# AssemblyAI-Community/MinImagen

Hardware: NVIDIA H100
Metric: denoising steps/sec (SR256 U-Net, batch 32 per GPU per step) (higher is better)
Workload: dtype f16 tensor-core operands, f32 accumulate / residual stream

## Files before the change

### minimagen_b200/csrc/conv_tc.cu

```cuda
#include "conv_tc.cuh"

#include <cuda_runtime.h>
#include <mutex>
#include <stdio.h>

#include "kernels.cuh"
#include "launch.cuh"
#include "ptx.cuh"
#include "sat_half.cuh"
#include "wgmma.cuh"

namespace mi {

namespace {

constexpr int kNumThreads = 384;
constexpr uint32_t kABytes = kConvBlockM * kConvBlockK * 2;
constexpr uint32_t kRingBudget = 192 * 1024;
constexpr uint32_t kAuxBytes = 512;
constexpr uint32_t kSmemMax = 227 * 1024;
constexpr int kProducerRegs = 40;
constexpr int kConsumerRegs = 232;
static_assert(128 * kProducerRegs + 256 * kConsumerRegs <= 65536, "register file overcommitted");

template <int BLOCK_N>
struct Cfg {
    static constexpr uint32_t kBBytes = BLOCK_N * kConvBlockK * 2;
    static constexpr uint32_t kStageBytes = kABytes + kBBytes;
    static constexpr int kStages = (kRingBudget / kStageBytes) > 8 ? 8 : (kRingBudget / kStageBytes);
    static constexpr uint32_t kSmemBytes = kStages * kStageBytes + 1024  + kAuxBytes;
};

__device__ __forceinline__ float silu(float v) { return __fdividef(v, 1.0f + __expf(-v)); }

template <int BLOCK_N, bool GN>
__global__ void __launch_bounds__(kNumThreads, 1)
conv_wg_kernel(const __grid_constant__ CUtensorMap tmA, const __grid_constant__ CUtensorMap tmA2,
               const __grid_constant__ CUtensorMap tmB, const __grid_constant__ CUtensorMap tmX,
               const __grid_constant__ CUtensorMap tmX2, const __grid_constant__ ConvTcArgs args,
               const __grid_constant__ GnPrologueArgs gn) {
    using C = Cfg<BLOCK_N>;
    constexpr int STAGES = C::kStages;
    static_assert(2 * STAGES * 8 <= 256, "barrier block overlaps the GroupNorm scratch");

    extern __shared__ uint8_t smem_raw[];
    uint8_t* smem = reinterpret_cast<uint8_t*>((reinterpret_cast<uintptr_t>(smem_raw) + 1023) & ~uintptr_t(1023));
    uint64_t* bars = reinterpret_cast<uint64_t*>(smem + STAGES * C::kStageBytes);
    uint64_t* full_bar = bars;
    uint64_t* empty_bar = bars + STAGES;

    const int warp = threadIdx.x >> 5;
    const int lane = threadIdx.x & 31;
    const int wg = threadIdx.x >> 7;
    int* err = args.err_flag;

    if (threadIdx.x == 0) {
        ptx::prefetch_tensormap(&tmB);
        if (!GN) {
            ptx::prefetch_tensormap(&tmA);
            ptx::prefetch_tensormap(&tmA2);
        }
        for (int i = 0; i < STAGES; ++i) {
            ptx::mbar_init(&full_bar[i], GN ? 5 : 1);
            ptx::mbar_init(&empty_bar[i], 2);
        }
        ptx::fence_barrier_init();
    }
    __syncthreads();
    pdl_wait();

    const int num_tap_kb = args.num_taps * args.chunks_per_tap;
    const int num_kb = num_tap_kb + args.x_chunks;
    const int tiles_m = args.tiles_w * args.tiles_h * args.tiles_b;
    const int total_tiles = tiles_m * args.tiles_n;
    const int BW = 1 << args.bw_log2, BH = 1 << args.bh_log2;
    const int BB = kConvBlockM >> (args.bw_log2 + args.bh_log2);

    if (wg == 0) {
        if constexpr (!GN) {
            ptx::setmaxnreg_dec<kProducerRegs>();
            if (warp == 0) {
                int stage = 0;
                uint32_t phase = 0;
                for (int tile = blockIdx.x; tile < total_tiles; tile += gridDim.x) {
                    const int nt = tile % args.tiles_n;
                    const int mt = tile / args.tiles_n;
                    const int w0 = (mt % args.tiles_w) * BW;
                    const int h0 = ((mt / args.tiles_w) % args.tiles_h) * BH;
                    const int b0 = (mt / (args.tiles_w * args.tiles_h)) * BB;
                    const int n0 = nt * BLOCK_N;
                    for (int kb = 0; kb < num_kb; ++kb) {
                        ptx::mbar_wait(&empty_bar[stage], phase ^ 1, err, 100 + stage);
                        if (ptx::elect_one()) {
                            uint8_t* sa = smem + stage * C::kStageBytes;
                            uint8_t* sb = sa + kABytes;
                            ptx::mbar_arrive_expect_tx(&full_bar[stage], C::kStageBytes);
                            if (kb < num_tap_kb) {
                                const int t = kb / args.chunks_per_tap, j = kb - t * args.chunks_per_tap;
                                const int cw = w0 * args.in_stride + args.dw[t], ch = h0 * args.in_stride + args.dh[t];
                                if (j < args.a_split)
                                    ptx::tma_load_5d(&tmA, &full_bar[stage], sa, args.a_chan_off + j * kConvBlockK, cw, ch,
                                                     args.ph[t], b0);
                                else
                                    ptx::tma_load_5d(&tmA2, &full_bar[stage], sa,
                                                     args.a_chan_off2 + (j - args.a_split) * kConvBlockK, cw, ch, args.ph[t], b0);
                            } else {
                                const int jx = kb - num_tap_kb;
                                if (jx < args.x_split)
                                    ptx::tma_load_5d(&tmX, &full_bar[stage], sa, args.x_chan_off + jx * kConvBlockK, w0, h0, 0, b0);
                                else
                                    ptx::tma_load_5d(&tmX2, &full_bar[stage], sa,
                                                     args.x_chan_off2 + (jx - args.x_split) * kConvBlockK, w0, h0, 0, b0);
                            }
                            ptx::tma_load_2d(&tmB, &full_bar[stage], sb, kb * kConvBlockK, n0);
                        }
                        if (++stage == STAGES) { stage = 0; phase ^= 1; }
                    }
                }
                pdl_trigger();
            }
        } else {
            float* s_mean = reinterpret_cast<float*>(reinterpret_cast<uint8_t*>(bars) + 256);
            float* s_rstd = s_mean + 32;
            float* sA = reinterpret_cast<float*>(reinterpret_cast<uint8_t*>(bars) + kAuxBytes);
            const int tt = threadIdx.x;
            const int lq = tt & 7;
            const int prow = tt >> 3;
            const int C0 = gn.C0, C1 = gn.C1, Ctot = C0 + C1, Cg = Ctot / gn.groups;
            const int H = args.H, W = args.W;
            float* sB = sA + Ctot;
            int stage = 0;
            uint32_t phase = 0;
            int cur_b = -1;
            for (int tile = blockIdx.x; tile < total_tiles; tile += gridDim.x) {
                const int nt = tile % args.tiles_n;
                const int mt = tile / args.tiles_n;
                const int w0 = (mt % args.tiles_w) * BW;
                const int h0 = ((mt / args.tiles_w) % args.tiles_h) * BH;
                const int b = mt / (args.tiles_w * args.tiles_h);
                const int n0 = nt * BLOCK_N;
                if (b != cur_b) {
                    ptx::bar_sync(1, 128);
                    if (tt < gn.groups) {
                        const int g = tt;
                        double su = 0.0, sq = 0.0;
                        const int lo = g * Cg, hi = lo + Cg;
                        const int lo0 = min(lo, C0), hi0 = min(hi, C0);
                        for (int e = lo0 / 16; e < hi0 / 16; ++e) {
                            su += gn.stats0[((long long)b * (C0 / 16) + e) * 2];
                            sq += gn.stats0[((long long)b * (C0 / 16) + e) * 2 + 1];
                        }
                        const int lo1 = max(lo, C0) - C0, hi1 = max(hi, C0) - C0;
                        for (int e = lo1 / 16; e < hi1 / 16; ++e) {
                            su += (double)gn.scale1 * gn.stats1[((long long)b * (C1 / 16) + e) * 2];
                            sq += (double)gn.scale1 * (double)gn.scale1 * gn.stats1[((long long)b * (C1 / 16) + e) * 2 + 1];
                        }
                        const double n = (double)Cg * H * W;
                        const double mean = su / n;
                        double var = sq / n - mean * mean;
                        if (var < 0) var = 0;
                        s_mean[g] = (float)mean;
                        s_rstd[g] = (float)(1.0 / sqrt(var + (double)gn.eps));
                    }
                    ptx::bar_sync(1, 128);
                    for (int cc = tt; cc < Ctot; cc += 128) {
                        const int g = cc / Cg;
                        float a = s_rstd[g] * gn.gamma[cc];
                        float bb = gn.beta[cc] - s_mean[g] * a;
                        if (gn.scale_shift) {
                            const float sc = gn.scale_shift[(long long)b * gn.ss_ld + cc] + 1.0f;
                            const float shv = gn.scale_shift[(long long)b * gn.ss_ld + Ctot + cc];
                            a *= sc;
                            bb = bb * sc + shv;
                        }
                        if (cc >= C0) a *= gn.scale1;
                        sA[cc] = a;
                        sB[cc] = bb;
                    }
                    cur_b = b;
                    ptx::bar_sync(1, 128);
                }
                const long long img = (long long)b * H * W;
                for (int kb = 0; kb < num_kb; ++kb) {
                    const int t = kb / args.chunks_per_tap, j = kb - t * args.chunks_per_tap;
                    const int dh = args.dh[t], dw = args.dw[t];
                    const float* cA = sA + j * kConvBlockK + lq * 8;
                    const float* cB = sB + j * kConvBlockK + lq * 8;
                    const float4 a0 = *reinterpret_cast<const float4*>(cA), a1 = *reinterpret_cast<const float4*>(cA + 4);
                    const float4 b0 = *reinterpret_cast<const float4*>(cB), b1 = *reinterpret_cast<const float4*>(cB + 4);
                    const bool first = j < args.a_split;
                    const int Cs = first ? C0 : C1;
                    const float* src = (first ? gn.src0 + (long long)j * kConvBlockK
                                              : gn.src1 + (long long)(j - args.a_split) * kConvBlockK) + img * Cs + lq * 8;

                    ptx::mbar_wait(&empty_bar[stage], phase ^ 1, err, 600 + stage);
                    uint8_t* sa = smem + stage * C::kStageBytes;
                    if (warp == 0 && ptx::elect_one()) {
                        ptx::mbar_arrive_expect_tx(&full_bar[stage], C::kBBytes);
                        ptx::tma_load_2d(&tmB, &full_bar[stage], sa + kABytes, kb * kConvBlockK, n0);
                    }
                    float4 x0[8], x1[8];
                    bool ok[8];
#pragma unroll
                    for (int i = 0; i < 8; ++i) {
                        const int m = i * 16 + prow;
                        const int gw = w0 + (m & (BW - 1)) + dw;
                        const int gh = h0 + ((m >> args.bw_log2) & (BH - 1)) + dh;
                        ok[i] = gh >= 0 && gh < H && gw >= 0 && gw < W;
                        if (ok[i]) {
                            const float4* s4 = reinterpret_cast<const float4*>(src + ((long long)gh * W + gw) * Cs);
                            x0[i] = __ldg(s4);
                            x1[i] = __ldg(s4 + 1);
                        }
                    }
#pragma unroll
                    for (int i = 0; i < 8; ++i) {
                        const int m = i * 16 + prow;
                        uint4 o = make_uint4(0u, 0u, 0u, 0u);
                        if (ok[i]) {
                            const __half2 h0_ = sat_half2(silu(fmaf(x0[i].x, a0.x, b0.x)), silu(fmaf(x0[i].y, a0.y, b0.y)));
                            const __half2 h1_ = sat_half2(silu(fmaf(x0[i].z, a0.z, b0.z)), silu(fmaf(x0[i].w, a0.w, b0.w)));
                            const __half2 h2_ = sat_half2(silu(fmaf(x1[i].x, a1.x, b1.x)), silu(fmaf(x1[i].y, a1.y, b1.y)));
                            const __half2 h3_ = sat_half2(silu(fmaf(x1[i].z, a1.z, b1.z)), silu(fmaf(x1[i].w, a1.w, b1.w)));
                            o.x = *reinterpret_cast<const uint32_t*>(&h0_); o.y = *reinterpret_cast<const uint32_t*>(&h1_);
                            o.z = *reinterpret_cast<const uint32_t*>(&h2_); o.w = *reinterpret_cast<const uint32_t*>(&h3_);
                        }
                        *reinterpret_cast<uint4*>(sa + m * 128 + ((lq ^ (m & 7)) << 4)) = o;
                    }
                    ptx::fence_proxy_async_smem();
                    __syncwarp();
                    if (lane == 0) ptx::mbar_arrive(&full_bar[stage]);
                    if (++stage == STAGES) { stage = 0; phase ^= 1; }
                }
            }
            pdl_trigger();
        }
    } else {
        if constexpr (!GN) ptx::setmaxnreg_inc<kConsumerRegs>();
        const int cw = wg - 1;
        const int wq = warp & 3;
        const int cq = 2 * (lane & 3);
        float acc[BLOCK_N / 2];
        int stage = 0;
        uint32_t phase = 0;
        int m_r[2], bw_r[2], bh_r[2], bb_r[2];
#pragma unroll
        for (int r = 0; r < 2; ++r) {
            m_r[r] = cw * 64 + wq * 16 + (lane >> 2) + 8 * r;
            bw_r[r] = m_r[r] & (BW - 1);
            bh_r[r] = (m_r[r] >> args.bw_log2) & (BH - 1);
            bb_r[r] = m_r[r] >> (args.bw_log2 + args.bh_log2);
        }
        const int m_warp = cw * 64 + wq * 16;
        const int bb_warp = m_warp >> (args.bw_log2 + args.bh_log2);
        const bool vec = args.out_sc == 1 && ((reinterpret_cast<uintptr_t>(args.out_f32) & 7) == 0) &&
                         ((reinterpret_cast<uintptr_t>(args.residual) & 7) == 0) &&
                         ((reinterpret_cast<uintptr_t>(args.out_f16) & 3) == 0);

        for (int tile = blockIdx.x; tile < total_tiles; tile += gridDim.x) {
            const int nt = tile % args.tiles_n;
            const int mt = tile / args.tiles_n;
            const int n0 = nt * BLOCK_N;
            int prev = -1;
            for (int kb = 0; kb < num_kb; ++kb) {
                ptx::mbar_wait(&full_bar[stage], phase, err, 300 + stage);
                const uint32_t sa = ptx::smem_u32(smem + stage * C::kStageBytes);
                const uint64_t da = ptx::make_sw128_desc(sa + cw * (64 * 128));
                const uint64_t db = ptx::make_sw128_desc(sa + kABytes);
                ptx::wg_fence();
#pragma unroll
                for (int k = 0; k < kConvBlockK / 16; ++k)
                    ptx::Wgmma<BLOCK_N, 0>::run(acc, da + 2 * k, db + 2 * k, (kb | k) != 0);
                ptx::wg_commit();
                ptx::wg_wait<1>();
                if (prev >= 0 && (threadIdx.x & 127) == 0) ptx::mbar_arrive(&empty_bar[prev]);
                prev = stage;
                if (++stage == STAGES) { stage = 0; phase ^= 1; }
            }
            ptx::wg_wait<0>();
            ptx::wg_fence_regs(acc);
            if (prev >= 0 && (threadIdx.x & 127) == 0) ptx::mbar_arrive(&empty_bar[prev]);

            const int tw0 = (mt % args.tiles_w) * BW;
            const int th0 = ((mt / args.tiles_w) % args.tiles_h) * BH;
            const int tb0 = (mt / (args.tiles_w * args.tiles_h)) * BB;
            bool valid[2];
            long long pix[2];
#pragma unroll
            for (int r = 0; r < 2; ++r) {
                const int w = tw0 + bw_r[r], h = th0 + bh_r[r], b = tb0 + bb_r[r];
                valid[r] = (b < args.B) && (h < args.H) && (w < args.W);
                pix[r] = (long long)b * args.out_sb + (long long)h * args.out_sh + (long long)w * args.out_sw;
            }
            const bool fast = vec && n0 + BLOCK_N <= args.n_valid;
            float st_s[BLOCK_N / 16 > 0 ? BLOCK_N / 16 : 1], st_q[BLOCK_N / 16 > 0 ? BLOCK_N / 16 : 1];
#pragma unroll
            for (int q = 0; q < BLOCK_N / 16; ++q) { st_s[q] = 0.f; st_q[q] = 0.f; }
#pragma unroll
            for (int j = 0; j < BLOCK_N / 8; ++j) {
                const int n = n0 + 8 * j + cq;
                if (fast) {
                    float2 bv = make_float2(0.f, 0.f);
                    if (args.bias) bv = __ldg(reinterpret_cast<const float2*>(args.bias + n));
#pragma unroll
                    for (int r = 0; r < 2; ++r) {
                        if (!valid[r]) continue;
                        const long long o = pix[r] + n;
                        float2 f = make_float2(acc[4 * j + 2 * r] + bv.x, acc[4 * j + 2 * r + 1] + bv.y);
                        if (args.residual) {
                            const float2 rv = *reinterpret_cast<const float2*>(args.residual + o);
                            f.x += rv.x; f.y += rv.y;
                        }
                        st_s[j >> 1] += f.x + f.y;
                        st_q[j >> 1] += f.x * f.x + f.y * f.y;
                        if (args.out_f32) *reinterpret_cast<float2*>(args.out_f32 + o) = f;
                        if (args.out_f16) *reinterpret_cast<__half2*>(args.out_f16 + o) = sat_half2(f.x, f.y);
                    }
                } else {
#pragma unroll
                    for (int r = 0; r < 2; ++r) {
#pragma unroll
                        for (int e = 0; e < 2; ++e) {
                            if (!valid[r] || n + e >= args.n_valid) continue;
                            float f = acc[4 * j + 2 * r + e] + (args.bias ? __ldg(args.bias + n + e) : 0.f);
                            const long long o = pix[r] + (long long)(n + e) * args.out_sc;
                            if (args.residual && args.out_sc == 1) f += args.residual[o];
                            st_s[j >> 1] += f;
                            st_q[j >> 1] += f * f;
                            if (args.out_f32) args.out_f32[o] = f;
                            if (args.out_f16) args.out_f16[o] = sat_half(f);
                        }
                    }
                }
            }
            if (args.stats) {
                const int b_img = tb0 + bb_warp;
                const bool any = __any_sync(0xffffffffu, valid[0] || valid[1]);
#pragma unroll
                for (int q = 0; q < BLOCK_N / 16; ++q) {
#pragma unroll
                    for (int o = 1; o <= 16; o <<= 1) {
                        st_s[q] += __shfl_xor_sync(0xffffffffu, st_s[q], o);
                        st_q[q] += __shfl_xor_sync(0xffffffffu, st_q[q], o);
                    }
                    if (lane == 0 && any) {
                        double* dst = args.stats + ((long long)b_img * args.stats_blocks + (n0 >> 4) + q) * 2;
                        atomicAdd(dst, (double)st_s[q]);
                        atomicAdd(dst + 1, (double)st_q[q]);
                    }
                }
            }
        }
    }
}


typedef CUresult (*PFN_encodeTiled)(CUtensorMap*, CUtensorMapDataType, cuuint32_t, void*, const cuuint64_t*,
                                    const cuuint64_t*, const cuuint32_t*, const cuuint32_t*, CUtensorMapInterleave,
                                    CUtensorMapSwizzle, CUtensorMapL2promotion, CUtensorMapFloatOOBfill);

PFN_encodeTiled get_encode() {
    static PFN_encodeTiled fn = nullptr;
    static std::once_flag once;
    std::call_once(once, [] {
        void* p = nullptr;
        cudaDriverEntryPointQueryResult q;
        if (cudaGetDriverEntryPoint("cuTensorMapEncodeTiled", &p, cudaEnableDefault, &q) == cudaSuccess &&
            q == cudaDriverEntryPointSuccess)
            fn = reinterpret_cast<PFN_encodeTiled>(p);
    });
    return fn;
}

int ilog2_exact(int v) {
    int l = 0;
    while ((1 << l) < v) ++l;
    return ((1 << l) == v) ? l : -1;
}

int num_sms_of_current_device() {
    int dev = 0;
    cudaGetDevice(&dev);
    static int cache[64] = {0};
    if (dev < 64 && cache[dev] != 0) return cache[dev];
    int n = 0;
    cudaDeviceGetAttribute(&n, cudaDevAttrMultiProcessorCount, dev);
    if (dev < 64) cache[dev] = n;
    return n;
}

void tile_geometry(int H, int W, int B, ConvTcArgs& a) {
    int BW = W >= 128 ? 128 : W;
    int BH = 128 / BW;
    if (BH > H) BH = H;
    const int BB = 128 / (BW * BH);
    a.bw_log2 = ilog2_exact(BW);
    a.bh_log2 = ilog2_exact(BH);
    a.tiles_w = (W + BW - 1) / BW;
    a.tiles_h = H / BH;
    a.tiles_b = (B + BB - 1) / BB;
    a.B = B; a.H = H; a.W = W;
}

int pick_block_n(int Cout, int tiles_m, int hint, int num_sms) {
    const int cands[5] = {256, 128, 64, 32, 16};
    if (hint < 0) hint = -hint;
    if (hint > 0 && Cout % hint == 0)
        for (int i = 0; i < 5; ++i)
            if (cands[i] == hint) return hint;
    int block_n = 16;
    for (int i = 0; i < 5; ++i) {
        if (Cout % cands[i] != 0) continue;
        block_n = cands[i];
        if (tiles_m * (Cout / cands[i]) >= num_sms || cands[i] <= 64) break;
    }
    return block_n;
}

CUresult encode_act(PFN_encodeTiled enc, CUtensorMap* m, const void* ptr, cuuint64_t channels, cuuint64_t ld, int W, int H,
                    int phases, int B, int in_stride, const ConvTcArgs& a) {
    const cuuint64_t IS = in_stride;
    const int BW = 1 << a.bw_log2, BH = 1 << a.bh_log2, BB = kConvBlockM >> (a.bw_log2 + a.bh_log2);
    cuuint64_t gdim[5] = {channels, (cuuint64_t)W * IS, (cuuint64_t)H * IS, (cuuint64_t)phases, (cuuint64_t)B};
    cuuint64_t gstr[4] = {ld * 2, (cuuint64_t)W * IS * ld * 2, (cuuint64_t)H * IS * W * IS * ld * 2,
                          (cuuint64_t)phases * H * IS * W * IS * ld * 2};
    cuuint32_t box[5] = {kConvBlockK, (cuuint32_t)(BW * IS), (cuuint32_t)(BH * IS), 1, (cuuint32_t)BB};
    cuuint32_t estr[5] = {1, (cuuint32_t)IS, (cuuint32_t)IS, 1, 1};
    return enc(m, CU_TENSOR_MAP_DATA_TYPE_FLOAT16, 5, const_cast<void*>(ptr), gdim, gstr, box, estr,
               CU_TENSOR_MAP_INTERLEAVE_NONE, CU_TENSOR_MAP_SWIZZLE_128B, CU_TENSOR_MAP_L2_PROMOTION_L2_256B,
               CU_TENSOR_MAP_FLOAT_OOB_FILL_NONE);
}

CUresult encode_weights(PFN_encodeTiled enc, CUtensorMap* m, const void* ptr, cuuint64_t K, int Cout, int block_n) {
    cuuint64_t gdim[2] = {K, (cuuint64_t)Cout};
    cuuint64_t gstr[1] = {K * 2};
    cuuint32_t box[2] = {kConvBlockK, (cuuint32_t)block_n};
    cuuint32_t estr[2] = {1, 1};
    return enc(m, CU_TENSOR_MAP_DATA_TYPE_FLOAT16, 2, const_cast<void*>(ptr), gdim, gstr, box, estr,
               CU_TENSOR_MAP_INTERLEAVE_NONE, CU_TENSOR_MAP_SWIZZLE_128B, CU_TENSOR_MAP_L2_PROMOTION_L2_256B,
               CU_TENSOR_MAP_FLOAT_OOB_FILL_NONE);
}

template <int BLOCK_N, bool GN>
int launch(const CUtensorMap& tmA, const CUtensorMap& tmA2, const CUtensorMap& tmB, const CUtensorMap& tmX,
           const CUtensorMap& tmX2, const ConvTcArgs& args, const GnPrologueArgs& gn, uint32_t extra_smem,
           cudaStream_t stream) {
    using C = Cfg<BLOCK_N>;
    static bool attr_set = false;
    if (!attr_set) {
        if (cudaFuncSetAttribute(conv_wg_kernel<BLOCK_N, GN>, cudaFuncAttributeMaxDynamicSharedMemorySize, kSmemMax) !=
            cudaSuccess)
            return -10;
        attr_set = true;
    }
    const int total_tiles = args.tiles_w * args.tiles_h * args.tiles_b * args.tiles_n;
    const int num_sms = num_sms_of_current_device();
    const int grid = total_tiles < num_sms ? total_tiles : num_sms;
    launch_k(conv_wg_kernel<BLOCK_N, GN>, grid, kNumThreads, C::kSmemBytes + extra_smem, stream, tmA, tmA2, tmB, tmX, tmX2,
             args, gn);
    return cudaGetLastError() == cudaSuccess ? 0 : -11;
}

}

PFN_tmaEncodeTiled get_tma_encode() { return get_encode(); }

const char* conv_tc_strerror(int code) {
    switch (code) {
        case 0: return "ok";
        case -1: return "conv_tc: C_in (per tap) must be a positive multiple of 64";
        case -2: return "conv_tc: C_out must be a multiple of 16";
        case -3: return "conv_tc: W must be a power of two >= 8 or a multiple of 128; H*W tiling unsupported";
        case -4: return "conv_tc: too many taps (max 16)";
        case -5: return "conv_tc: cuTensorMapEncodeTiled unavailable";
        case -6: return "conv_tc: tensor map encode failed (activations)";
        case -7: return "conv_tc: tensor map encode failed (weights)";
        case -8: return "conv_tc: pointer/stride alignment (16 B) violated";
        case -9: return "conv_tc: the folded 1x1 operand needs a stride-1 conv over one phase";
        case -10: return "conv_tc: cudaFuncSetAttribute(max dynamic smem) failed";
        case -11: return "conv_tc: kernel launch failed";
        default: return "conv_tc: unknown error";
    }
}

bool conv_tc_supported(int H, int W, int Cin, int Cout) {
    if (Cin <= 0 || Cin % kConvBlockK != 0 || Cout <= 0 || Cout % 16 != 0) return false;
    if (W >= 128) return true;
    if (ilog2_exact(W) < 3) return false;
    const int bh = 128 / W;
    if (H >= bh) return H % bh == 0;
    return ilog2_exact(H) >= 0;
}

int conv_tc_launch(const ConvTcProblem& p, cudaStream_t stream) {
    if (p.Cin <= 0 || p.Cin % kConvBlockK != 0) return -1;
    if (p.Cout % 16 != 0) return -2;
    if (p.num_taps < 1 || p.num_taps > kConvMaxTaps) return -4;
    if (!conv_tc_supported(p.H, p.W, p.Cin, p.Cout)) return -3;
    if ((reinterpret_cast<uintptr_t>(p.act) & 15) || (reinterpret_cast<uintptr_t>(p.wpacked) & 15) ||
        (p.lda % 8) != 0)
        return -8;
    PFN_encodeTiled enc = get_encode();
    if (!enc) return -5;

    ConvTcArgs a{};
    a.num_taps = p.num_taps;
    a.chunks_per_tap = p.Cin / kConvBlockK;
    tile_geometry(p.H, p.W, p.B, a);
    a.a_chan_off = p.a_chan_off;
    a.in_stride = p.in_stride == 2 ? 2 : 1;
    a.out_sb = p.out_sb; a.out_sh = p.out_sh; a.out_sw = p.out_sw;
    a.out_sc = p.out_sc > 0 ? p.out_sc : 1;
    a.n_valid = p.n_valid > 0 ? p.n_valid : p.Cout;
    a.out_f32 = p.out_f32; a.out_f16 = p.out_f16; a.bias = p.bias; a.residual = p.residual;
    a.err_flag = p.err_flag;
    a.stats = p.stats; a.stats_blocks = p.Cout / 16;
    for (int t = 0; t < p.num_taps; ++t) { a.dh[t] = p.dh[t]; a.dw[t] = p.dw[t]; a.ph[t] = p.ph[t]; }

    const int tiles_m = a.tiles_w * a.tiles_h * a.tiles_b;
    const int block_n = pick_block_n(p.Cout, tiles_m, p.block_n_hint, num_sms_of_current_device());
    a.tiles_n = p.Cout / block_n;

    CUtensorMap tmA, tmA2, tmB, tmX, tmX2;
    a.a_split = (p.act2 ? p.Cin1 : p.Cin) / kConvBlockK;
    a.a_chan_off2 = p.a_chan_off2;
    if (encode_act(enc, &tmA, p.act, p.a_channels, p.lda, p.W, p.H, p.phases, p.B, a.in_stride, a) != CUDA_SUCCESS) return -6;
    tmA2 = tmA;
    if (p.act2) {
        if (p.Cin1 <= 0 || p.Cin1 % kConvBlockK || p.Cin1 >= p.Cin || (p.lda2 % 8) || (reinterpret_cast<uintptr_t>(p.act2) & 15) ||
            a.in_stride != 1)
            return -8;
        if (encode_act(enc, &tmA2, p.act2, p.lda2, p.lda2, p.W, p.H, p.phases, p.B, 1, a) != CUDA_SUCCESS) return -6;
    }
    tmX = tmA; tmX2 = tmA;
    if (p.x_act) {
        if (p.phases != 1 || a.in_stride != 1) return -9;
        if (p.Cx <= 0 || p.Cx % kConvBlockK || (p.x_lda % 8) || (reinterpret_cast<uintptr_t>(p.x_act) & 15)) return -8;
        if (p.x_act2 && (p.Cx1 <= 0 || p.Cx1 % kConvBlockK || p.Cx1 >= p.Cx || (p.x_lda2 % 8) ||
                         (reinterpret_cast<uintptr_t>(p.x_act2) & 15)))
            return -8;
        a.x_chunks = p.Cx / kConvBlockK;
        a.x_split = (p.x_act2 ? p.Cx1 : p.Cx) / kConvBlockK;
        a.x_chan_off = p.x_chan_off; a.x_chan_off2 = p.x_chan_off2;
        if (encode_act(enc, &tmX, p.x_act, p.x_lda, p.x_lda, p.W, p.H, 1, p.B, 1, a) != CUDA_SUCCESS) return -6;
        tmX2 = tmX;
        if (p.x_act2 && encode_act(enc, &tmX2, p.x_act2, p.x_lda2, p.x_lda2, p.W, p.H, 1, p.B, 1, a) != CUDA_SUCCESS) return -6;
    }
    const cuuint64_t K = (cuuint64_t)p.num_taps * p.Cin + (p.x_act ? (cuuint64_t)p.Cx : 0);
    if (encode_weights(enc, &tmB, p.wpacked, K, p.Cout, block_n) != CUDA_SUCCESS) return -7;

    const GnPrologueArgs gn{};
    switch (block_n) {
        case 256: return launch<256, false>(tmA, tmA2, tmB, tmX, tmX2, a, gn, 0, stream);
        case 128: return launch<128, false>(tmA, tmA2, tmB, tmX, tmX2, a, gn, 0, stream);
        case 64: return launch<64, false>(tmA, tmA2, tmB, tmX, tmX2, a, gn, 0, stream);
        case 32: return launch<32, false>(tmA, tmA2, tmB, tmX, tmX2, a, gn, 0, stream);
        default: return launch<16, false>(tmA, tmA2, tmB, tmX, tmX2, a, gn, 0, stream);
    }
}


bool conv_gn_supported(int H, int W, int C0, int C1, int Cout, int groups) {
    const int C = C0 + C1;
    if (H <= 0 || W <= 0 || H % 32 || W % 8 || C0 <= 0 || C0 % 64 || C1 < 0 || C1 % 64 || Cout <= 0 || Cout % 128) return false;
    if (!conv_tc_supported(H, W, C, Cout) || H * W < kConvBlockM) return false;
    if (groups < 1 || groups > 32 || C % groups) return false;
    if (Cfg<128>::kSmemBytes + 8u * (uint32_t)C > kSmemMax) return false;
    return (C / groups) % 16 == 0;
}

int conv_gn_launch(const ConvGnProblem& p, cudaStream_t stream) {
    if (!conv_gn_supported(p.H, p.W, p.C0, p.C1, p.Cout, p.groups)) return -3;
    if (p.C1 && (!p.src1 || !p.stats1)) return -8;
    if (!p.src0 || !p.stats0 || !p.gamma || !p.beta) return -8;
    if ((reinterpret_cast<uintptr_t>(p.src0) & 15) || (reinterpret_cast<uintptr_t>(p.src1) & 15) ||
        (reinterpret_cast<uintptr_t>(p.wpacked) & 15))
        return -8;
    PFN_encodeTiled enc = get_encode();
    if (!enc) return -5;
    const int C = p.C0 + p.C1;

    ConvTcArgs a{};
    a.num_taps = 9;
    for (int t = 0; t < 9; ++t) { a.dh[t] = (int8_t)(t / 3 - 1); a.dw[t] = (int8_t)(t % 3 - 1); a.ph[t] = 0; }
    a.chunks_per_tap = C / kConvBlockK;
    a.a_split = p.C0 / kConvBlockK;
    a.in_stride = 1;
    tile_geometry(p.H, p.W, p.B, a);
    a.out_sb = (long long)p.H * p.W * p.Cout; a.out_sh = (long long)p.W * p.Cout; a.out_sw = p.Cout; a.out_sc = 1;
    a.n_valid = p.Cout;
    a.out_f32 = p.out_f32; a.out_f16 = p.out_f16; a.bias = p.bias; a.residual = p.residual; a.err_flag = p.err_flag;
    a.stats = p.out_stats; a.stats_blocks = p.Cout / 16;
    a.tiles_n = p.Cout / 128;

    GnPrologueArgs g{};
    g.src0 = p.src0; g.src1 = p.src1;
    g.C0 = p.C0; g.C1 = p.C1; g.groups = p.groups; g.scale1 = p.scale1; g.eps = p.eps;
    g.stats0 = p.stats0; g.stats1 = p.stats1; g.gamma = p.gamma; g.beta = p.beta;
    g.scale_shift = p.scale_shift; g.ss_ld = p.ss_ld;

    CUtensorMap tmB;
    if (encode_weights(enc, &tmB, p.wpacked, (cuuint64_t)9 * C, p.Cout, 128) != CUDA_SUCCESS) return -7;
    return launch<128, true>(tmB, tmB, tmB, tmB, tmB, a, g, 8u * (uint32_t)C, stream);
}

}
```

### minimagen_b200/csrc/ptx.cuh

```cuda
#pragma once
#include <cuda.h>
#include <cuda_fp16.h>
#include <stdint.h>

namespace mi {
namespace ptx {

__device__ __forceinline__ uint32_t smem_u32(const void* p) {
    return static_cast<uint32_t>(__cvta_generic_to_shared(p));
}

__device__ __forceinline__ void mbar_init(uint64_t* bar, uint32_t count) {
    asm volatile("mbarrier.init.shared::cta.b64 [%0], %1;" ::"r"(smem_u32(bar)), "r"(count));
}
__device__ __forceinline__ void fence_barrier_init() {
    asm volatile("fence.mbarrier_init.release.cluster;" ::: "memory");
}
__device__ __forceinline__ void fence_proxy_async_smem() {
    asm volatile("fence.proxy.async.shared::cta;" ::: "memory");
}
__device__ __forceinline__ void mbar_arrive(uint64_t* bar) {
    asm volatile("mbarrier.arrive.shared::cta.b64 _, [%0];" ::"r"(smem_u32(bar)) : "memory");
}
__device__ __forceinline__ void mbar_arrive_expect_tx(uint64_t* bar, uint32_t bytes) {
    asm volatile("mbarrier.arrive.expect_tx.shared::cta.b64 _, [%0], %1;" ::"r"(smem_u32(bar)), "r"(bytes)
                 : "memory");
}
__device__ __forceinline__ bool mbar_try_wait(uint64_t* bar, uint32_t parity) {
    uint32_t ok;
    asm volatile(
        "{\n\t"
        ".reg .pred p;\n\t"
        "mbarrier.try_wait.parity.shared::cta.b64 p, [%1], %2;\n\t"
        "selp.u32 %0, 1, 0, p;\n\t"
        "}"
        : "=r"(ok)
        : "r"(smem_u32(bar)), "r"(parity)
        : "memory");
    return ok != 0;
}
__device__ __forceinline__ void mbar_wait(uint64_t* bar, uint32_t parity, int* err, int code) {
    if (mbar_try_wait(bar, parity)) return;
    const long long t0 = clock64();
    while (!mbar_try_wait(bar, parity)) {
        if (clock64() - t0 > 4000000000LL) {
            if (err) { atomicExch(err, code); __threadfence_system(); }
            __trap();
        }
    }
}

__device__ __forceinline__ bool elect_one() {
    uint32_t pred;
    asm volatile("{\n .reg .pred p;\n elect.sync _|p, 0xffffffff;\n selp.u32 %0, 1, 0, p;\n}" : "=r"(pred));
    return pred != 0;
}

__device__ __forceinline__ float ex2_approx(float x) {
    float y;
    asm("ex2.approx.ftz.f32 %0, %1;" : "=f"(y) : "f"(x));
    return y;
}

__device__ __forceinline__ int ld_acquire_gpu(const int* p) {
    int v;
    asm volatile("ld.acquire.gpu.global.s32 %0, [%1];" : "=r"(v) : "l"(p) : "memory");
    return v;
}

__device__ __forceinline__ void prefetch_tensormap(const CUtensorMap* m) {
    asm volatile("prefetch.tensormap [%0];" ::"l"(reinterpret_cast<uint64_t>(m)) : "memory");
}
__device__ __forceinline__ void tma_load_2d(const CUtensorMap* m, uint64_t* bar, void* dst, int c0, int c1) {
    asm volatile(
        "cp.async.bulk.tensor.2d.shared::cluster.global.mbarrier::complete_tx::bytes [%0], [%1, {%3, %4}], [%2];"
        ::"r"(smem_u32(dst)), "l"(reinterpret_cast<uint64_t>(m)), "r"(smem_u32(bar)), "r"(c0), "r"(c1)
        : "memory");
}
__device__ __forceinline__ void tma_load_5d(const CUtensorMap* m, uint64_t* bar, void* dst, int c0, int c1, int c2,
                                            int c3, int c4) {
    asm volatile(
        "cp.async.bulk.tensor.5d.shared::cluster.global.mbarrier::complete_tx::bytes [%0], [%1, {%3, %4, %5, %6, "
        "%7}], [%2];"
        ::"r"(smem_u32(dst)), "l"(reinterpret_cast<uint64_t>(m)), "r"(smem_u32(bar)), "r"(c0), "r"(c1), "r"(c2),
        "r"(c3), "r"(c4)
        : "memory");
}

__device__ __forceinline__ void wg_fence() { asm volatile("wgmma.fence.sync.aligned;" ::: "memory"); }
__device__ __forceinline__ void wg_commit() { asm volatile("wgmma.commit_group.sync.aligned;" ::: "memory"); }
template <int N>
__device__ __forceinline__ void wg_wait() { asm volatile("wgmma.wait_group.sync.aligned %0;" ::"n"(N) : "memory"); }
template <int R>
__device__ __forceinline__ void wg_fence_regs(float (&d)[R]) {
#pragma unroll
    for (int i = 0; i < R; ++i) asm volatile("" : "+f"(d[i])::"memory");
}

__device__ __forceinline__ uint64_t make_sw128_desc(uint32_t smem_addr, uint32_t lbo_bytes = 16) {
    uint64_t d = 0;
    d |= static_cast<uint64_t>((smem_addr >> 4) & 0x3FFF);
    d |= static_cast<uint64_t>((lbo_bytes >> 4) & 0x3FFF) << 16;
    d |= static_cast<uint64_t>(1024u >> 4) << 32;
    d |= static_cast<uint64_t>(1) << 62;
    return d;
}
__device__ __forceinline__ void bar_sync(int id, int count) {
    asm volatile("bar.sync %0, %1;" ::"r"(id), "r"(count) : "memory");
}

template <int N>
__device__ __forceinline__ void setmaxnreg_dec() { asm volatile("setmaxnreg.dec.sync.aligned.u32 %0;" ::"n"(N)); }
template <int N>
__device__ __forceinline__ void setmaxnreg_inc() { asm volatile("setmaxnreg.inc.sync.aligned.u32 %0;" ::"n"(N)); }

}
}
```

Measured before the change: 11.73.

## Ping-pong consumer warpgroups across tiles so epilogue overlaps the other's MMA

For non-GroupNorm convs with BLOCK_N up to 128, each consumer warpgroup now computes the full 128-row tile, with two accumulator halves, on alternating tiles. Named barriers hand the tensor cores back and forth, so one warpgroup's epilogue (bias, residual, stores, stats) overlaps the other's wgmma mainloop. The empty barrier count drops to one, and each warpgroup skips the ring stages consumed by its partner. GroupNorm stats are also reduced per tile through shared-memory scratch before the double atomics, which cuts atomic traffic. In exchange the accumulator register footprint doubles, which risks spills at 232 registers, and the cross-warpgroup ordering adds synchronisation complexity.

```diff
diff --git a/minimagen_b200/csrc/conv_tc.cu b/minimagen_b200/csrc/conv_tc.cu
--- a/minimagen_b200/csrc/conv_tc.cu
+++ b/minimagen_b200/csrc/conv_tc.cu
@@ -22,6 +22,9 @@
 constexpr int kProducerRegs = 40;
 constexpr int kConsumerRegs = 232;
 static_assert(128 * kProducerRegs + 256 * kConsumerRegs <= 65536, "register file overcommitted");
+constexpr int kTurnBar = 2;
+constexpr int kStatBar = 4;
+constexpr uint32_t stat_scratch_bytes(int block_n) { return 2 * 4 * (block_n / 16 > 0 ? block_n / 16 : 1) * 2 * 8; }
 
 template <int BLOCK_N>
 struct Cfg {
@@ -42,6 +45,8 @@
     using C = Cfg<BLOCK_N>;
     constexpr int STAGES = C::kStages;
     static_assert(2 * STAGES * 8 <= 256, "barrier block overlaps the GroupNorm scratch");
+    constexpr bool PP = !GN && BLOCK_N <= 128;
+    constexpr int HALVES = PP ? 2 : 1;
 
     extern __shared__ uint8_t smem_raw[];
     uint8_t* smem = reinterpret_cast<uint8_t*>((reinterpret_cast<uintptr_t>(smem_raw) + 1023) & ~uintptr_t(1023));
@@ -62,7 +67,7 @@
         }
         for (int i = 0; i < STAGES; ++i) {
             ptx::mbar_init(&full_bar[i], GN ? 5 : 1);
-            ptx::mbar_init(&empty_bar[i], 2);
+            ptx::mbar_init(&empty_bar[i], PP ? 1 : 2);
         }
         ptx::fence_barrier_init();
     }
@@ -240,115 +245,155 @@
         const int cw = wg - 1;
         const int wq = warp & 3;
         const int cq = 2 * (lane & 3);
-        float acc[BLOCK_N / 2];
+        float acc[HALVES][BLOCK_N / 2];
         int stage = 0;
         uint32_t phase = 0;
-        int m_r[2], bw_r[2], bh_r[2], bb_r[2];
-#pragma unroll
-        for (int r = 0; r < 2; ++r) {
-            m_r[r] = cw * 64 + wq * 16 + (lane >> 2) + 8 * r;
-            bw_r[r] = m_r[r] & (BW - 1);
-            bh_r[r] = (m_r[r] >> args.bw_log2) & (BH - 1);
-            bb_r[r] = m_r[r] >> (args.bw_log2 + args.bh_log2);
+        auto skip = [&](int n) {
+            stage += n % STAGES;
+            phase ^= (uint32_t)(n / STAGES) & 1u;
+            if (stage >= STAGES) { stage -= STAGES; phase ^= 1; }
+        };
+        if (PP) skip(cw * num_kb);
+        int bw_r[2 * HALVES], bh_r[2 * HALVES], bb_r[2 * HALVES], bb_warp[HALVES];
+#pragma unroll
+        for (int h = 0; h < HALVES; ++h) {
+            const int m_warp = (PP ? h : cw) * 64 + wq * 16;
+            bb_warp[h] = m_warp >> (args.bw_log2 + args.bh_log2);
+#pragma unroll
+            for (int r = 0; r < 2; ++r) {
+                const int m = m_warp + (lane >> 2) + 8 * r;
+                bw_r[2 * h + r] = m & (BW - 1);
+                bh_r[2 * h + r] = (m >> args.bw_log2) & (BH - 1);
+                bb_r[2 * h + r] = m >> (args.bw_log2 + args.bh_log2);
+            }
         }
-        const int m_warp = cw * 64 + wq * 16;
-        const int bb_warp = m_warp >> (args.bw_log2 + args.bh_log2);
+        constexpr int NQ = BLOCK_N / 16 > 0 ? BLOCK_N / 16 : 1;
+        const bool tile_stats = PP && args.stats != nullptr && BB == 1;
+        double* st_red = reinterpret_cast<double*>(reinterpret_cast<uint8_t*>(bars) + kAuxBytes);
         const bool vec = args.out_sc == 1 && ((reinterpret_cast<uintptr_t>(args.out_f32) & 7) == 0) &&
                          ((reinterpret_cast<uintptr_t>(args.residual) & 7) == 0) &&
                          ((reinterpret_cast<uintptr_t>(args.out_f16) & 3) == 0);
 
-        for (int tile = blockIdx.x; tile < total_tiles; tile += gridDim.x) {
+        for (int tile = blockIdx.x + (PP ? cw : 0) * gridDim.x; tile < total_tiles; tile += (PP ? 2 : 1) * gridDim.x) {
             const int nt = tile % args.tiles_n;
             const int mt = tile / args.tiles_n;
             const int n0 = nt * BLOCK_N;
+            if (PP && tile != (int)blockIdx.x) ptx::bar_sync(kTurnBar + cw, 256);
             int prev = -1;
             for (int kb = 0; kb < num_kb; ++kb) {
                 ptx::mbar_wait(&full_bar[stage], phase, err, 300 + stage);
                 const uint32_t sa = ptx::smem_u32(smem + stage * C::kStageBytes);
-                const uint64_t da = ptx::make_sw128_desc(sa + cw * (64 * 128));
                 const uint64_t db = ptx::make_sw128_desc(sa + kABytes);
                 ptx::wg_fence();
 #pragma unroll
                 for (int k = 0; k < kConvBlockK / 16; ++k)
-                    ptx::Wgmma<BLOCK_N, 0>::run(acc, da + 2 * k, db + 2 * k, (kb | k) != 0);
+#pragma unroll
+                    for (int h = 0; h < HALVES; ++h) {
+                        const uint64_t da = ptx::make_sw128_desc(sa + (PP ? h : cw) * (64 * 128));
+                        ptx::Wgmma<BLOCK_N, 0>::run(acc[h], da + 2 * k, db + 2 * k, (kb | k) != 0);
+                    }
                 ptx::wg_commit();
                 ptx::wg_wait<1>();
                 if (prev >= 0 && (threadIdx.x & 127) == 0) ptx::mbar_arrive(&empty_bar[prev]);
                 prev = stage;
                 if (++stage == STAGES) { stage = 0; phase ^= 1; }
             }
+            if (PP && tile + (int)gridDim.x < total_tiles) ptx::bar_arrive(kTurnBar + (cw ^ 1), 256);
+            if (PP) skip(num_kb);
             ptx::wg_wait<0>();
-            ptx::wg_fence_regs(acc);
+#pragma unroll
+            for (int h = 0; h < HALVES; ++h) ptx::wg_fence_regs(acc[h]);
             if (prev >= 0 && (threadIdx.x & 127) == 0) ptx::mbar_arrive(&empty_bar[prev]);
 
             const int tw0 = (mt % args.tiles_w) * BW;
             const int th0 = ((mt / args.tiles_w) % args.tiles_h) * BH;
             const int tb0 = (mt / (args.tiles_w * args.tiles_h)) * BB;
-            bool valid[2];
-            long long pix[2];
-#pragma unroll
-            for (int r = 0; r < 2; ++r) {
-                const int w = tw0 + bw_r[r], h = th0 + bh_r[r], b = tb0 + bb_r[r];
-                valid[r] = (b < args.B) && (h < args.H) && (w < args.W);
-                pix[r] = (long long)b * args.out_sb + (long long)h * args.out_sh + (long long)w * args.out_sw;
-            }
             const bool fast = vec && n0 + BLOCK_N <= args.n_valid;
-            float st_s[BLOCK_N / 16 > 0 ? BLOCK_N / 16 : 1], st_q[BLOCK_N / 16 > 0 ? BLOCK_N / 16 : 1];
-#pragma unroll
-            for (int q = 0; q < BLOCK_N / 16; ++q) { st_s[q] = 0.f; st_q[q] = 0.f; }
-#pragma unroll
-            for (int j = 0; j < BLOCK_N / 8; ++j) {
-                const int n = n0 + 8 * j + cq;
-                if (fast) {
-                    float2 bv = make_float2(0.f, 0.f);
-                    if (args.bias) bv = __ldg(reinterpret_cast<const float2*>(args.bias + n));
-#pragma unroll
-                    for (int r = 0; r < 2; ++r) {
-                        if (!valid[r]) continue;
-                        const long long o = pix[r] + n;
-                        float2 f = make_float2(acc[4 * j + 2 * r] + bv.x, acc[4 * j + 2 * r + 1] + bv.y);
-                        if (args.residual) {
-                            const float2 rv = *reinterpret_cast<const float2*>(args.residual + o);
-                            f.x += rv.x; f.y += rv.y;
-                        }
-                        st_s[j >> 1] += f.x + f.y;
-                        st_q[j >> 1] += f.x * f.x + f.y * f.y;
-                        if (args.out_f32) *reinterpret_cast<float2*>(args.out_f32 + o) = f;
-                        if (args.out_f16) *reinterpret_cast<__half2*>(args.out_f16 + o) = sat_half2(f.x, f.y);
-                    }
-                } else {
-#pragma unroll
-                    for (int r = 0; r < 2; ++r) {
-#pragma unroll
-                        for (int e = 0; e < 2; ++e) {
-                            if (!valid[r] || n + e >= args.n_valid) continue;
-                            float f = acc[4 * j + 2 * r + e] + (args.bias ? __ldg(args.bias + n + e) : 0.f);
-                            const long long o = pix[r] + (long long)(n + e) * args.out_sc;
-                            if (args.residual && args.out_sc == 1) f += args.residual[o];
-                            st_s[j >> 1] += f;
-                            st_q[j >> 1] += f * f;
-                            if (args.out_f32) args.out_f32[o] = f;
-                            if (args.out_f16) args.out_f16[o] = sat_half(f);
+#pragma unroll
+            for (int hf = 0; hf < HALVES; ++hf) {
+                bool valid[2];
+                long long pix[2];
+#pragma unroll
+                for (int r = 0; r < 2; ++r) {
+                    const int w = tw0 + bw_r[2 * hf + r], h = th0 + bh_r[2 * hf + r], b = tb0 + bb_r[2 * hf + r];
+                    valid[r] = (b < args.B) && (h < args.H) && (w < args.W);
+                    pix[r] = (long long)b * args.out_sb + (long long)h * args.out_sh + (long long)w * args.out_sw;
+                }
+                const float* a = acc[hf];
+                float st_s[BLOCK_N / 16 > 0 ? BLOCK_N / 16 : 1], st_q[BLOCK_N / 16 > 0 ? BLOCK_N / 16 : 1];
+#pragma unroll
+                for (int q = 0; q < BLOCK_N / 16; ++q) { st_s[q] = 0.f; st_q[q] = 0.f; }
+#pragma unroll
+                for (int j = 0; j < BLOCK_N / 8; ++j) {
+                    const int n = n0 + 8 * j + cq;
+                    if (fast) {
+                        float2 bv = make_float2(0.f, 0.f);
+                        if (args.bias) bv = __ldg(reinterpret_cast<const float2*>(args.bias + n));
+#pragma unroll
+                        for (int r = 0; r < 2; ++r) {
+                            if (!valid[r]) continue;
+                            const long long o = pix[r] + n;
+                            float2 f = make_float2(a[4 * j + 2 * r] + bv.x, a[4 * j + 2 * r + 1] + bv.y);
+                            if (args.residual) {
+                                const float2 rv = *reinterpret_cast<const float2*>(args.residual + o);
+                                f.x += rv.x; f.y += rv.y;
+                            }
+                            st_s[j >> 1] += f.x + f.y;
+                            st_q[j >> 1] += f.x * f.x + f.y * f.y;
+                            if (args.out_f32) *reinterpret_cast<float2*>(args.out_f32 + o) = f;
+                            if (args.out_f16) *reinterpret_cast<__half2*>(args.out_f16 + o) = sat_half2(f.x, f.y);
+                        }
+                    } else {
+#pragma unroll
+                        for (int r = 0; r < 2; ++r) {
+#pragma unroll
+                            for (int e = 0; e < 2; ++e) {
+                                if (!valid[r] || n + e >= args.n_valid) continue;
+                                float f = a[4 * j + 2 * r + e] + (args.bias ? __ldg(args.bias + n + e) : 0.f);
+                                const long long o = pix[r] + (long long)(n + e) * args.out_sc;
+                                if (args.residual && args.out_sc == 1) f += args.residual[o];
+                                st_s[j >> 1] += f;
+                                st_q[j >> 1] += f * f;
+                                if (args.out_f32) args.out_f32[o] = f;
+                                if (args.out_f16) args.out_f16[o] = sat_half(f);
+                            }
+                        }
+                    }
+                }
+                if (args.stats) {
+                    const int b_img = tb0 + bb_warp[hf];
+                    const bool any = __any_sync(0xffffffffu, valid[0] || valid[1]);
+#pragma unroll
+                    for (int q = 0; q < BLOCK_N / 16; ++q) {
+#pragma unroll
+                        for (int o = 1; o <= 16; o <<= 1) {
+                            st_s[q] += __shfl_xor_sync(0xffffffffu, st_s[q], o);
+                            st_q[q] += __shfl_xor_sync(0xffffffffu, st_q[q], o);
+                        }
+                        if (lane == 0 && tile_stats) {
+                            double* r = st_red + ((cw * 4 + wq) * NQ + q) * 2;
+                            r[0] = (hf == 0 ? 0.0 : r[0]) + (double)st_s[q];
+                            r[1] = (hf == 0 ? 0.0 : r[1]) + (double)st_q[q];
+                        } else if (lane == 0 && any) {
+                            double* dst = args.stats + ((long long)b_img * args.stats_blocks + (n0 >> 4) + q) * 2;
+                            atomicAdd(dst, (double)st_s[q]);
+                            atomicAdd(dst + 1, (double)st_q[q]);
                         }
                     }
                 }
             }
-            if (args.stats) {
-                const int b_img = tb0 + bb_warp;
-                const bool any = __any_sync(0xffffffffu, valid[0] || valid[1]);
-#pragma unroll
-                for (int q = 0; q < BLOCK_N / 16; ++q) {
-#pragma unroll
-                    for (int o = 1; o <= 16; o <<= 1) {
-                        st_s[q] += __shfl_xor_sync(0xffffffffu, st_s[q], o);
-                        st_q[q] += __shfl_xor_sync(0xffffffffu, st_q[q], o);
-                    }
-                    if (lane == 0 && any) {
-                        double* dst = args.stats + ((long long)b_img * args.stats_blocks + (n0 >> 4) + q) * 2;
-                        atomicAdd(dst, (double)st_s[q]);
-                        atomicAdd(dst + 1, (double)st_q[q]);
-                    }
+            if (tile_stats) {
+                ptx::bar_sync(kStatBar + cw, 128);
+                if (wq == 0 && lane < NQ) {
+                    const double* r = st_red + (cw * 4 * NQ + lane) * 2;
+                    double s = r[0], sq = r[1];
+#pragma unroll
+                    for (int w = 1; w < 4; ++w) { s += r[w * NQ * 2]; sq += r[w * NQ * 2 + 1]; }
+                    double* dst = args.stats + ((long long)tb0 * args.stats_blocks + (n0 >> 4) + lane) * 2;
+                    atomicAdd(dst, s);
+                    atomicAdd(dst + 1, sq);
                 }
+                ptx::bar_sync(kStatBar + cw, 128);
             }
         }
     }
@@ -456,8 +501,8 @@
     const int total_tiles = args.tiles_w * args.tiles_h * args.tiles_b * args.tiles_n;
     const int num_sms = num_sms_of_current_device();
     const int grid = total_tiles < num_sms ? total_tiles : num_sms;
-    launch_k(conv_wg_kernel<BLOCK_N, GN>, grid, kNumThreads, C::kSmemBytes + extra_smem, stream, tmA, tmA2, tmB, tmX, tmX2,
-             args, gn);
+    const uint32_t smem = C::kSmemBytes + (!GN && BLOCK_N <= 128 ? stat_scratch_bytes(BLOCK_N) : 0u) + extra_smem;
+    launch_k(conv_wg_kernel<BLOCK_N, GN>, grid, kNumThreads, smem, stream, tmA, tmA2, tmB, tmX, tmX2, args, gn);
     return cudaGetLastError() == cudaSuccess ? 0 : -11;
 }
 
diff --git a/minimagen_b200/csrc/ptx.cuh b/minimagen_b200/csrc/ptx.cuh
--- a/minimagen_b200/csrc/ptx.cuh
+++ b/minimagen_b200/csrc/ptx.cuh
@@ -108,6 +108,9 @@
 __device__ __forceinline__ void bar_sync(int id, int count) {
     asm volatile("bar.sync %0, %1;" ::"r"(id), "r"(count) : "memory");
 }
+__device__ __forceinline__ void bar_arrive(int id, int count) {
+    asm volatile("bar.arrive %0, %1;" ::"r"(id), "r"(count) : "memory");
+}
 
 template <int N>
 __device__ __forceinline__ void setmaxnreg_dec() { asm volatile("setmaxnreg.dec.sync.aligned.u32 %0;" ::"n"(N)); }
```

Result: faster. 12.17 (median of 6 runs) (+3.7%).
